# Meowuu7/equi-articulated-pose

Hardware: AMD Instinct MI355X
Metric: point-clouds/sec (4096 pts, 60 anchors) fwd+bwd (higher is better)
Workload: dtype f32; 1 GPU; 8 x 4096-pt synthetic laptop clouds per GPU, 3-block inter backbone 1->64->128->512 (NN=64,K=24,A=60), forward+backward+Adam; clouds_per_gpu=8, points=4096, anchors=60

## Files before the change

equi-articulated-pose_amd/csrc/gemm_bf16x3.hip:

```cpp
#include "common.h"
#include "device_prims.h"
#include <algorithm>
#include <type_traits>

namespace {

constexpr int BK = 16, BN = 256;
constexpr unsigned PLANE_BYTES = 256 * BK * 2;
constexpr unsigned oper_bytes(int pl) { return (unsigned)pl * PLANE_BYTES; }
constexpr unsigned stage_bytes(int pl) { return 2 * oper_bytes(pl); }
constexpr size_t shmem_bytes(int pl) { return 3 * (size_t)stage_bytes(pl); }
constexpr int WAVES_N = 4;

struct Args {
    int M, N, K;
    const float *A; long long lda;
    const float *B; long long ldb, sB;
    float *C; long long ldc, sC;
    int tiles_m, tiles_n;
    const int *tbl; int na;
    int nr;
    const unsigned *Apre;
    long long sA; int slabs, kslab;
    const float *ep_scale, *ep_shift, *ep_res; float ep_slope; long long sRes;
// ... 46 lines not shown

    int id = blockIdx.x, tm, tn;
    {
        const int groups = g.tiles_n / 8 * 8;
        const int xcd = id & 7, slot = id >> 3;
        const int panel = (slot / g.tiles_m) * 8 + xcd;
        if (panel < groups && id < groups * g.tiles_m) { tn = panel; tm = slot % g.tiles_m; }
        else { const int r = id - groups * g.tiles_m; tn = groups + r / g.tiles_m; tm = r % g.tiles_m; }
    }
    const int z = blockIdx.y;
    const int m0 = tm * BM, n0 = tn * BN;
    const int item = g.slabs > 1 ? z / g.slabs : z;
    const long long item_of_z = item;
    const long long kbeg = g.slabs > 1 ? (long long)(z - item * g.slabs) * g.kslab : 0;
    const float *A = g.A + item * g.sA + kbeg;
    const float *B = g.B + item * g.sB + (BMODE == 0 ? kbeg : 0);
    float *C = g.C + (long long)z * g.sC;

    const int t = threadIdx.x, lane = t & 63;
    const int wave = __builtin_amdgcn_readfirstlane(t >> 6);
    const int wm = wave / WN, wn = wave % WN;
    const int li = lane & 31, lh = lane >> 5;

    const int c4 = t & 3, rq = t >> 2;
    const int c4b = BMODE ? __builtin_amdgcn_readfirstlane(t >> 7) : c4, rqb = BMODE ? (t & 127) : rq;
    const float *baseA[NPA], *baseB[NPO];
#pragma unroll
    for (int u = 0; u < NPA; ++u) baseA[u] = A + (long long)min(m0 + RG * u, g.M - RG) * g.lda;
#pragma unroll
    for (int u = 0; u < NPO; ++u) baseB[u] = B + (long long)min(n0 + RG * u, g.N - RG) * g.ldb;
    const unsigned char *preA[NPA];
    constexpr int PRE_PIECE = PL == 3 ? 32 : 16;
    const long long pre_pitch = (long long)(g.K / 4) * PRE_PIECE;
#pragma unroll
    for (int u = 0; u < NPA; ++u) preA[u] = reinterpret_cast<const unsigned char *>(g.Apre) + (long long)min(m0 + RG * u, g.M - RG) * pre_pitch;
    const unsigned offP = (unsigned)((long long)rq * pre_pitch + PRE_PIECE * c4);
    float sclA[2] = {1.0f, 1.0f}, sclB[2] = {1.0f, 1.0f};
    const unsigned *absBz = g.absB + item_of_z * g.sAbsB;
    if constexpr (PL == 2) {
#pragma unroll
        for (int u = 0; u < NPA; ++u) sclA[u] = pow2_scale(__uint_as_float(g.absA[min(m0 + RG * u, g.M - RG) + rq]));
#pragma unroll
        for (int u = 0; u < NPO; ++u) sclB[u] = pow2_scale(__uint_as_float(absBz[(min(n0 + RG * u, g.N - RG) + rqb) / g.grpB]) * g.multB);
    }
    const unsigned offA = (unsigned)((long long)rq * g.lda + 4 * c4) * 4u, offB = (unsigned)((long long)rq * g.ldb + 4 * c4) * 4u;
    unsigned colB[NPO], tapB[NPO];
#pragma unroll
    for (int u = 0; u < NPO; ++u) {
        const int n = min(n0 + RG * u, g.N - RG) + rqb;
        if constexpr (BMODE == 2) {
// ... 314 lines not shown
void keep_pool_memory() {
    static bool done[64] = {};
    int dev = 0;
    if (hipGetDevice(&dev) != hipSuccess || dev < 0 || dev >= 64 || done[dev]) return;
    done[dev] = true;
    hipMemPool_t pool;
    if (hipDeviceGetDefaultMemPool(&pool, dev) == hipSuccess) {
        uint64_t keep = ~0ull;
        (void)hipMemPoolSetAttribute(pool, hipMemPoolAttrReleaseThreshold, &keep);
    }
    (void)hipGetLastError();
}

template <int BMODE, int PL = 3>
int launch_split(Args &g, long long batch, hipStream_t stream, const char *who) {
    bool pre = g.sA == 0 && g.slabs <= 1 && (g_presplit == 2 || (g_presplit == 1 && g.K >= 1024));
    void *scratch = nullptr;
    if (pre) {
        const long long pieces = (long long)g.M * (g.K / 4);
        keep_pool_memory();
        if (hipMallocAsync(&scratch, (size_t)pieces * (PL == 3 ? 32 : 16), stream) != hipSuccess) {
            (void)hipGetLastError();
            scratch = nullptr;
            pre = false;
        }
    }
    struct Release {
        void *p; hipStream_t s;
        ~Release() { if (p) (void)hipFreeAsync(p, s); }
    } release{scratch, stream};
    if (pre) {
// ... 281 lines not shown
    if (!eap_gemm_bf16x3_reduce_f32_supported(M, N, K, A, lda, strideA, B, ldb, strideB, ldc) || (reinterpret_cast<uintptr_t>(C) & 15) ||
        (reinterpret_cast<uintptr_t>(workspace) & 15))
        return eap::bad_arg("gemm_bf16x3_reduce_f32: unsupported operands (ask eap_gemm_bf16x3_reduce_f32_supported)");
    const int slabs = reduce_slabs(M, N, K, batch);
    Args g{};
    g.M = M; g.N = N; g.K = K;
    g.A = A; g.lda = lda; g.sA = strideA;
    g.B = B; g.ldb = ldb; g.sB = strideB;
    g.C = workspace; g.ldc = N; g.sC = (long long)M * N;
    g.slabs = slabs; g.kslab = K / slabs;
    if (int e = launch_split<0>(g, (long long)batch * slabs, eap::S(stream), "gemm_bf16x3_reduce_f32")) return e;
    const long long mn4 = (long long)M * N / 4;
    return eap::run_kernel("gemm_bf16x3_reduce_f32 (sum of the partials)", split_reduce_kernel, eap::cdiv(mn4, 256), 1, 1, dim3(256), 0, eap::S(stream), mn4,
                           batch * slabs, reinterpret_cast<const f32x4 *>(workspace), C, N, (long long)ldc);
}
```

equi-articulated-pose_amd/csrc/grouping.hip:

```cpp
#include "common.h"

namespace {

constexpr int BQ_THREADS = 64;
constexpr int BQ_TILE = 1024;

__device__ __forceinline__ float add_rn(float a, float b) { return __fadd_rn(a, b); }
__device__ __forceinline__ double add_rn(double a, double b) { return __dadd_rn(a, b); }
__device__ __forceinline__ float sub_rn(float a, float b) { return __fsub_rn(a, b); }
__device__ __forceinline__ double sub_rn(double a, double b) { return __dsub_rn(a, b); }
__device__ __forceinline__ float mul_rn(float a, float b) { return __fmul_rn(a, b); }
__device__ __forceinline__ double mul_rn(double a, double b) { return __dmul_rn(a, b); }
__device__ __forceinline__ float div_rn(float a, float b) { return __fdiv_rn(a, b); }
__device__ __forceinline__ double div_rn(double a, double b) { return __ddiv_rn(a, b); }
__device__ __forceinline__ float sqrt_t(float a) { return sqrtf(a); }
__device__ __forceinline__ double sqrt_t(double a) { return sqrt(a); }
__device__ __forceinline__ float acos_t(float a) { return acosf(a); }
__device__ __forceinline__ double acos_t(double a) { return acos(a); }
__device__ __forceinline__ float min_t(float a, float b) { return fminf(a, b); }
__device__ __forceinline__ double min_t(double a, double b) { return fmin(a, b); }

template <typename T>
__device__ __forceinline__ T sq3(T x, T y, T z) {
    return add_rn(add_rn(mul_rn(x, x), mul_rn(y, y)), mul_rn(z, z));
// ... 1 lines not shown
template <typename T>
__device__ __forceinline__ T d2_exact(T ax, T ay, T az, T bx, T by, T bz) {
    return sq3(sub_rn(ax, bx), sub_rn(ay, by), sub_rn(az, bz));
}

template <typename T>
__global__ __launch_bounds__(BQ_THREADS) void ball_query_kernel(
    int n, int m, T radius2, int nsample, const T *__restrict__ new_xyz,
    const T *__restrict__ xyz, int32_t *__restrict__ idx) {
    __shared__ T tile[3][BQ_TILE];
    const int bi = blockIdx.y;
    xyz += (size_t)bi * 3 * n;
    new_xyz += (size_t)bi * 3 * m;
    idx += (size_t)bi * m * nsample;

    const int j = blockIdx.x * BQ_THREADS + threadIdx.x;
    const bool live = j < m;
    T qx = 0, qy = 0, qz = 0;
    if (live) { qx = new_xyz[j]; qy = new_xyz[m + j]; qz = new_xyz[2 * m + j]; }
    int32_t *out = idx + (size_t)(live ? j : 0) * nsample;

    int cnt = live ? 0 : nsample;
    for (int k0 = 0; k0 < n; k0 += BQ_TILE) {
        const int len = min(BQ_TILE, n - k0);
        __syncthreads();
        for (int t = threadIdx.x; t < len; t += BQ_THREADS) {
            tile[0][t] = xyz[k0 + t];
            tile[1][t] = xyz[n + k0 + t];
            tile[2][t] = xyz[2 * n + k0 + t];
        }
        __syncthreads();
        for (int t = 0; t < len && cnt < nsample; ++t) {
            const T d2 = d2_exact(qx, qy, qz, tile[0][t], tile[1][t], tile[2][t]);
            if (d2 < radius2) { out[cnt] = k0 + t; ++cnt; }
        }
        if (__syncthreads_and(cnt >= nsample)) break;
    }
    if (!live) return;
    if (cnt < nsample - 1) {
        if (cnt == 0) {
            for (int t = 0; t < nsample; ++t) out[t] = 0;
        } else {
            for (int t = cnt; t < nsample; ++t) out[t] = out[t - cnt];
        }
    } else if (cnt == nsample - 1) {
        out[nsample - 1] = 0;
    }
}

template <typename T>
int launch_ball_query(int b, int n, int m, float radius, int nsample, const T *new_xyz,
                      const T *xyz, int32_t *idx, hipStream_t s) {
    if (b <= 0 || m <= 0 || nsample <= 0) return 0;
    if (n <= 0) return eap::bad_arg("ball_query: empty support cloud");
    const T r2 = (T)(radius * radius);
    return eap::run_kernel("ball_query", ball_query_kernel<T>, eap::cdiv(m, BQ_THREADS), b, 1, dim3(BQ_THREADS), 0, s, n, m, r2, nsample, new_xyz, xyz, idx);
}


template <typename T>
__global__ __launch_bounds__(1024) void fps_kernel(int n, int m, const T *__restrict__ xyz,
                                                  T *__restrict__ temp, int32_t *__restrict__ idx) {
    __shared__ T s_d[1024];
    __shared__ int s_i[1024];
    const int bi = blockIdx.x, tid = threadIdx.x, nt = blockDim.x;
    xyz += (size_t)bi * 3 * n;
    temp += (size_t)bi * n;
    idx += (size_t)bi * m;
    for (int k = tid; k < n; k += nt) temp[k] = (T)1e10;
    int old = 0;
    if (tid == 0) idx[0] = 0;
// ... 148 lines not shown
```

equi-articulated-pose_amd/csrc/inv_lists.hip:

```cpp
#include "common.h"

namespace {

constexpr int RT = 1024;
constexpr int MAXN = 16384;

__global__ __launch_bounds__(256) void inv_count_kernel(int per_cloud, int n, const int32_t *__restrict__ idx,
                                                        int32_t *__restrict__ counts) {
    extern __shared__ int s_hist[];
    const int bi = blockIdx.y, t = threadIdx.x;
    for (int i = t; i < n; i += 256) s_hist[i] = 0;
    __syncthreads();
    const int chunk = (per_cloud + gridDim.x - 1) / gridDim.x;
    const int beg = blockIdx.x * chunk, end = min(per_cloud, beg + chunk);
    const int32_t *src = idx + (size_t)bi * per_cloud;
    for (int e = beg + t; e < end; e += 256) {
        const int q = src[e];
        if ((unsigned)q < (unsigned)n) atomicAdd(&s_hist[q], 1);
    }
    __syncthreads();
    for (int i = t; i < n; i += 256) {
        const int v = s_hist[i];
        if (v) atomicAdd(&counts[(size_t)bi * n + i], v);
    }
}

__global__ __launch_bounds__(RT) void inv_rows_kernel(int n, int n2, const int32_t *__restrict__ counts,
                                                      int32_t *__restrict__ rows, int32_t *__restrict__ off,
                                                      int32_t *__restrict__ cnt, int32_t *__restrict__ n_rows) {
    extern __shared__ unsigned long long s_key[];
    __shared__ int s_part[RT];
    const int bi = blockIdx.x, t = threadIdx.x;
    for (int i = t; i < n2; i += RT) {
        const unsigned c = i < n ? (unsigned)counts[(size_t)bi * n + i] : 0u;
        s_key[i] = c ? (((unsigned long long)c << 32) | (0xFFFFFFFFu - (unsigned)i)) : 0ull;
    }
    __syncthreads();
    for (int k = 2; k <= n2; k <<= 1) {
        for (int j = k >> 1; j > 0; j >>= 1) {
            for (int i = t; i < n2; i += RT) {
                const int l = i ^ j;
                if (l > i) {
                    const unsigned long long a = s_key[i], b = s_key[l];
                    const bool desc = (i & k) == 0;
                    if (desc ? a < b : a > b) { s_key[i] = b; s_key[l] = a; }
                }
            }
            __syncthreads();
        }
    }
    const int per = n2 / RT > 0 ? n2 / RT : 1;
    int local = 0, nz = 0;
    for (int u = 0; u < per; ++u) {
        const int i = t * per + u;
        if (i < n2) { const unsigned c = (unsigned)(s_key[i] >> 32); local += (int)c; nz += c != 0; }
    }
    s_part[t] = local;
    __syncthreads();
    for (int d = 1; d < RT; d <<= 1) {
        const int v = t >= d ? s_part[t - d] : 0;
        __syncthreads();
        s_part[t] += v;
        __syncthreads();
    }
    int run = s_part[t] - local;
    for (int u = 0; u < per; ++u) {
        const int i = t * per + u;
        if (i < n) {
            const unsigned long long key = s_key[i];
            const unsigned c = (unsigned)(key >> 32);
            rows[(size_t)bi * n + i] = c ? (int)(0xFFFFFFFFu - (unsigned)key) : -1;
            cnt[(size_t)bi * n + i] = (int)c;
            off[(size_t)bi * n + i] = run;
            run += (int)c;
        }
    }
    __syncthreads();
    s_part[t] = nz;
    __syncthreads();
    for (int d = RT / 2; d > 0; d >>= 1) {
        if (t < d) s_part[t] += s_part[t + d];
        __syncthreads();
    }
    if (t == 0) n_rows[bi] = s_part[0];
}

__global__ __launch_bounds__(256) void inv_fill_kernel(int per_cloud, int nn, int n, int rld,
                                                       const int32_t *__restrict__ idx, const float4 *__restrict__ gx,
                                                       const int32_t *__restrict__ rows, const int32_t *__restrict__ off,
                                                       int32_t *__restrict__ ent_p, float4 *__restrict__ ent_gx) {
    __shared__ int s_wave[4];
    const int r = blockIdx.x, bi = blockIdx.y;
    const int q = rows[(size_t)bi * rld + r];
    if (q < 0) return;
    const int t = threadIdx.x, lane = t & 63, wave = t >> 6;
    const int quads = per_cloud >> 2;
    const int qper = (quads + 3) / 4;
    const int qbeg = wave * qper, qend = min(quads, qbeg + qper);
    const int4 *src = reinterpret_cast<const int4 *>(idx + (size_t)bi * per_cloud);
// ... 106 lines not shown
```

equi-articulated-pose_amd/vgtk/_hip.py:

```python
import ctypes
import os
import re
import struct
import types
import weakref

import torch

_PKG_ROOT = os.path.abspath(os.path.join(os.path.dirname(__file__), '..'))
LIB_PATH = os.path.join(_PKG_ROOT, 'libeap_hip.so')

if not os.path.exists(LIB_PATH):
    raise ImportError(
        f'{LIB_PATH} not found: build the HIP extension first '
        '(python -c "import __graft_entry__ as g; g.build()" or make -C equi-articulated-pose_amd/csrc). '
        'This package has no CPU fallback.')

lib = ctypes.CDLL(LIB_PATH)


_HEADERS = (os.path.join(_PKG_ROOT, 'include', 'eap_hip.h'), os.path.join(os.path.dirname(_PKG_ROOT), 'include', 'eap_hip.h'))
HEADER_PATH = next((p for p in _HEADERS if os.path.exists(p)), _HEADERS[-1])

_I64 = ctypes.c_int64
# ... 255 lines not shown
def _product(A, B, out, reduce=False):
    ta, lda, sa, ba, M, K = operand(A, 'A')
    tb, ldb, sb, batch, Kb, N = operand(B, 'B')
    tc, ldc, sc, bc, Mc, Nc = operand(out, 'out')
    if B.dim() != 3 or out.dim() != 3 - reduce:
        raise RuntimeError(f'B is a stack of matrices, out {"one matrix" if reduce else "a stack"}: got B {tuple(B.shape)}, out {tuple(out.shape)}')
    if K != Kb or (M, N) != (Mc, Nc) or (A.dim() == 3 and ba != batch) or bc != (1 if reduce else batch):
        raise RuntimeError(f'A {tuple(A.shape)} x B {tuple(B.shape)} -> out {tuple(out.shape)}: the sizes do not agree')
    if tc:
        raise RuntimeError(f'out must be row-major (strides {tuple(out.stride())})')
    if (M > 1 and ldc < N) or (bc > 1 and sc < (M - 1) * ldc + N):
        raise RuntimeError(f'out {tuple(out.shape)} with strides {tuple(out.stride())} overlaps itself')
    return ta, tb, M, N, K, lda, sa, ldb, sb, ldc, sc, batch


def matmul(A, B, out, b_bound=None):
    ta, tb, M, N, K, lda, sa, ldb, sb, ldc, sc, batch = _product(A, B, out)
    gemm(ta, tb, M, N, K, A, lda, sa, B, ldb, sb, out, ldc, sc, batch, b_bound=b_bound)


def matmul_reduce(A, B, out):
    ta, tb, M, N, K, lda, sa, ldb, sb, ldc, _, batch = _product(A, B, out, reduce=True)
    gemm_reduce(ta, tb, M, N, K, A, lda, sa, B, ldb, sb, out, ldc, batch)


def matmul_reduce_takes_split(A, B, out):
    ta, tb, M, N, K, lda, sa, ldb, sb, ldc, _, _ = _product(A, B, out, reduce=True)
    return bool(SPLIT_BF16_CONTRACTION and not ta and tb and out.data_ptr() % 16 == 0 and
                abi.eap_gemm_bf16x3_reduce_f32_supported(M, N, K, A, lda, sa, B, ldb, sb, ldc))


def matmul_epilogue(A, B, out, scale, shift, slope, residual=None, b_bound=None):
# ... 346 lines not shown
    b, p, nn = idx.shape
    dev = idx.device
    wide = n > DENSE_NARROW_ROWS
    memb = torch.empty(b, p, 32 if wide else 16, dtype=torch.int32, device=dev)
    flags = torch.empty(b, dtype=torch.int32, device=dev)
    slot_of = torch.empty(b, n, dtype=torch.int32, device=dev)
    call('eap_so3_dense_member_wide' if wide else 'eap_so3_dense_member', idx, b, p, n, nn, min(DENSE_MAX_ROWS if wide else DENSE_NARROW_ROWS, n),
         rows.stride(0), idx, rows, n_rows, slot_of, memb, flags)
    return memb, flags


def so3_dense_narrow(memb, rp):
    if _dense_wide(memb) and rp <= DENSE_NARROW_ROWS:
        return memb[:, :, :16].contiguous()
    return memb


SORT_DENSE_POINTS = True
SKIP_DENSE_STEPS = True


class DenseGeometry:

    def __init__(self, q_xyz, s_xyz, memb, rows, rp, rk, sigma, nn, n_rows=None, row_rot=None, sort=None):
        b, p = memb.shape[:2]
        n = s_xyz.shape[2]
        na, ks, _ = rk.shape
        dev = memb.device
        memb = so3_dense_narrow(memb, rp)
        if memb.dtype != torch.int32 or not memb.is_contiguous() or memb.shape[2] not in (16, 32) or int(rp) > 32 * memb.shape[2]:
# ... 546 lines not shown
```

equi-articulated-pose_amd/vgtk/so3conv/functional.py:

```python
import math
import os
import weakref

import numpy as np
import torch

import vgtk
import vgtk.functional as fr
import vgtk.pc as pctk
import vgtk.spconv as zpconv
import vgtk.cuda.grouping as cuda_nn

from .. import _hip
from . import norm_fold

inter_so3conv_feat_grouping = zpconv.inter_zpconv_grouping_naive
batched_index_select = zpconv.batched_index_select
batched_index_select_other = zpconv.batched_index_select_other

MATERIALIZE_INTER_W = False

GAMMA_SIZE = 3
ROOT = vgtk.__path__[0]
Rs, R_idx, canonical_relative = fr.icosahedron_so3(GAMMA_SIZE)
# ... 360 lines not shown
    return ((bias.abs() > NORM_IN_NODE_MAX_RATIO * weight.abs()) & (weight != 0)).any().to(torch.int32)


class _ListHead:

    def __init__(self, idx, n_sup, nonident, gx=None, prefill=False, dense_probe=None, norm=None):
        dev = idx.device
        main = torch.cuda.current_stream(dev)
        side = _side_stream(dev)
        self.memb = None
        side.wait_stream(main)
        for t in (idx, gx, nonident) + tuple(x[1] if isinstance(x, tuple) else x for x in (dense_probe or ())):
            if t is not None:
                t.record_stream(side)
        ill = None
        if norm is not None:
            second = _side_stream(dev, True)
            second.wait_stream(main)
            with torch.cuda.stream(second):
                ill = _norm_ill(norm.weight.detach(), norm.bias.detach())
            ill.record_stream(side)
        with torch.cuda.stream(side):
            self.rows, self.off, self.cnt, self.n_rows = _hip.inv_lists_rows(idx, n_sup)
            flag = nonident.max() if nonident is not None else torch.ones((), dtype=torch.int32, device=dev)
            dense_bad = torch.ones((), dtype=torch.int32, device=dev)
            if dense_probe is not None:
                self.memb, dflags = _hip.so3_dense_member(idx, self.rows, self.n_rows, n_sup)
                dense_bad = dflags.max()
                eye = torch.eye(3, dtype=torch.float32, device=dev)
                for rot in dense_probe:
                    if isinstance(rot, tuple):
                        r = rot[1].double()
                        dense_bad = dense_bad + ((torch.matmul(r, r.transpose(-1, -2)) - eye.double()).abs().max() > 1e-6).to(torch.int32)
                    elif rot is not None:
                        dense_bad = dense_bad + (rot[:, :, :3, :3] != eye).any().to(torch.int32)
            groups16 = torch.zeros((), dtype=torch.int32, device=dev)
            if self.memb is not None:
                touched = ((self.memb & 0xffff) != 0).sum((1, 2)) + ((self.memb & -65536) != 0).sum((1, 2))
                groups16 = (touched.max().to(torch.float32) * (16.0 / max(idx.shape[1], 1))).to(torch.int32)
            stats = [self.n_rows.max().to(torch.int32), flag.to(torch.int32), dense_bad.to(torch.int32), groups16]
            if ill is not None:
                side.wait_stream(second)
                stats.append(ill)
            stats = torch.stack(stats)
            self.host = torch.empty(stats.shape[0], dtype=torch.int32, pin_memory=True)
            self.host.copy_(stats, non_blocking=True)
            self.entries = _hip.inv_lists_fill(idx, gx, self.rows, self.off, n_sup) if (prefill and gx is not None) else None
            self.event = torch.cuda.Event()
            self.event.record(side)
        for t in (self.rows, self.off, self.cnt, self.n_rows, self.memb) + (self.entries or ()):
            if t is not None:
                t.record_stream(main)

    def fill(self, idx, gx, n_sup):
        dev = idx.device
        main = torch.cuda.current_stream(dev)
        side = _side_stream(dev)
        with torch.cuda.stream(side):
            self.entries = _hip.inv_lists_fill(idx, gx, self.rows, self.off, n_sup)
            self.event = torch.cuda.Event()
            self.event.record(side)
        for t in self.entries:
            t.record_stream(main)

# ... 1248 lines not shown
```

include/eap_hip.h:

```cpp
#ifndef EAP_HIP_H
#define EAP_HIP_H

#include <stdint.h>

#ifdef __cplusplus
extern "C" {
#endif

typedef void *eap_stream_t;

const char *eap_last_error(void);
int eap_launch_dims_ok(int64_t gx, int64_t gy, int64_t gz, int bx, int by, int bz);
const char *eap_last_kernel(void);
int eap_abi_version(void);


int eap_ball_query_f32(int b, int n, int m, float radius, int nsample, const float *new_xyz,
                       const float *xyz, int32_t *idx, eap_stream_t stream);
int eap_ball_query_f64(int b, int n, int m, float radius, int nsample, const double *new_xyz,
                       const double *xyz, int32_t *idx, eap_stream_t stream);

int eap_furthest_point_sampling_f32(int b, int n, int m, const float *xyz, float *temp,
                                    int32_t *idx, eap_stream_t stream);
int eap_furthest_point_sampling_f64(int b, int n, int m, const double *xyz, double *temp,
// ... 193 lines not shown
                              const float *bound, float *scale, void *planes, eap_stream_t stream);
int eap_so3_dense_point_keys(int b, int p, const uint32_t *memb, int32_t *keys, eap_stream_t stream);
int64_t eap_so3_dense_steps_words(int b, int p, int ks, int rp, int dir);
int eap_so3_dense_steps(int b, int p, int ks, int rp, int dir, int skip, const int32_t *n_rows, const uint64_t *mask, int32_t *steps,
                        eap_stream_t stream);
int eap_so3_dense_product_steps_f32(int dir, int b, int o, int p, int na, int ks, int rp, int64_t ldz, float sigma, const int32_t *n_rows,
                                    const void *planes, const float *scale, const float *pt, const float *kr, const uint64_t *mask,
                                    const int32_t *steps, float *out, eap_stream_t stream);
int eap_so3_dense_max_rows(void);
int eap_so3_dense_member_wide(int b, int p, int n, int nn, int rp, int rows_ld, const int32_t *idx, const int32_t *rows,
                              const int32_t *n_rows, int32_t *slot_of, uint32_t *memb, int32_t *flags, eap_stream_t stream);
int eap_so3_dense_point_keys_wide(int b, int p, const uint32_t *memb, int64_t *keys, eap_stream_t stream);
int eap_so3_dense_masks_wide(int b, int p, int ks, int rp, int dir, const uint32_t *memb, uint64_t *mask, eap_stream_t stream);
int eap_so3_dense_steps_wide(int b, int p, int ks, int rp, int dir, int skip, const int32_t *n_rows, const uint64_t *mask, int32_t *steps,
                             eap_stream_t stream);


int eap_so3_intra_group_fwd_f32(int b, int c, int p, int na, int t, const float *feats,
                                const int32_t *intra_idx, float *out, eap_stream_t stream);
int eap_so3_intra_group_bwd_f32(int b, int c, int p, int na, int t, const float *gout,
                                const int32_t *intra_idx, float *gfeats, eap_stream_t stream);



int eap_gemm_f32(int transA, int transB, int M, int N, int K, const float *A, int64_t lda,
                 int64_t strideA, const float *B, int64_t ldb, int64_t strideB, float *C,
                 int64_t ldc, int64_t strideC, int batch, eap_stream_t stream);

int64_t eap_gemm_f32_reduce_workspace(int M, int N, int K, int batch);
int eap_gemm_f32_reduce(int transA, int transB, int M, int N, int K, const float *A, int64_t lda,
// ... 17 lines not shown
int64_t eap_gemm_bf16x3_reduce_workspace(int M, int N, int K, int batch);
int eap_gemm_bf16x3_reduce_f32(int M, int N, int K, const float *A, int64_t lda, int64_t strideA, const float *B, int64_t ldb,
                               int64_t strideB, float *C, int64_t ldc, int batch, float *workspace, eap_stream_t stream);
int eap_so3_intra_conv_bf16x3_f32_supported(int b, int o, int c, int p, int na, int nt);
int eap_so3_intra_conv_bf16x3_f32(int b, int o, int c, int p, int na, int nt, const float *W, const float *feats,
                                  const int32_t *intra_idx, float *out, eap_stream_t stream);
int eap_absmax_rows_f32(const float *x, int batch, int rows, int cols, int64_t ld, int64_t stride, int32_t *out_bits, eap_stream_t stream);
int eap_absmax_colgroups_f32(const float *x, int batch, int rows, int cols, int64_t ld, int64_t stride, int grp, int32_t *out_bits,
                             eap_stream_t stream);
int eap_so3_grouped_bound_f32(int b, int p, int nn, int n_sup, const int32_t *point_max_bits, const int32_t *idx, int32_t *out_bits,
                              eap_stream_t stream);
int eap_gemm_f16x2_f32(int trans_b, int M, int N, int K, const float *A, int64_t lda, const float *B, int64_t ldb, int64_t strideB,
                       float *C, int64_t ldc, int64_t strideC, int batch, const int32_t *abs_a, const int32_t *abs_b, int grp_b, float mult_b,
                       const float *scale, const float *shift, float slope, const float *residual, int64_t strideRes,
                       eap_stream_t stream);
int eap_so3_intra_conv_f16x2_f32(int b, int o, int c, int p, int na, int nt, const float *W, const float *feats,
                                 const int32_t *intra_idx, float *out, const int32_t *abs_w, const int32_t *abs_f, eap_stream_t stream);


int eap_gemm_dma_f32_supported(int transA, int transB, int M, int N, int K, const float *A, int64_t lda,
                               int64_t strideA, const float *B, int64_t ldb, int64_t strideB);
int eap_gemm_dma_f32(int transA, int transB, int M, int N, int K, const float *A, int64_t lda, int64_t strideA,
                     const float *B, int64_t ldb, int64_t strideB, float *C, int64_t ldc, int64_t strideC,
                     int batch, eap_stream_t stream);
int64_t eap_gemm_dma_f32_reduce_workspace(int M, int N, int K, int batch);
int eap_gemm_dma_f32_reduce(int transA, int transB, int M, int N, int K, const float *A, int64_t lda,
                            int64_t strideA, const float *B, int64_t ldb, int64_t strideB, float *C, int64_t ldc,
                            int batch, float *workspace, eap_stream_t stream);
int eap_gemm_skinny_reduce_f32_supported(int M, int N, int K, const float *A, int64_t lda, int64_t strideA, const float *B,
                                         int64_t ldb, int64_t strideB);
// ... 160 lines not shown
```

Measured before the change: 169.2 point-clouds/sec.

## Add split-K f16x2 GEMM, cooperative ball query, compact inverse-list sort, fused probe

Several unrelated changes land together. A split-K path for the two-plane GEMM with M=128 spreads the K dimension across slabs and sums the partials in a reduce kernel, so single-row-tile matmuls can fill the GPU. Ball query now uses 16 lanes per query with ballot-based compaction instead of one thread per query. The inverse-list sort compacts nonzero counts before a smaller bitonic sort, and a new native probe kernel folds several statistics checks into one pass on the side stream. The costs are an extra workspace and reduce launch, and changed ordering and fill semantics in ball query (out[t % cnt]).

```diff
diff --git a/equi-articulated-pose_amd/csrc/gemm_bf16x3.hip b/equi-articulated-pose_amd/csrc/gemm_bf16x3.hip
--- a/equi-articulated-pose_amd/csrc/gemm_bf16x3.hip
+++ b/equi-articulated-pose_amd/csrc/gemm_bf16x3.hip
@@ -84,8 +84,12 @@
     const long long item_of_z = item;
     const long long kbeg = g.slabs > 1 ? (long long)(z - item * g.slabs) * g.kslab : 0;
     const float *A = g.A + item * g.sA + kbeg;
-    const float *B = g.B + item * g.sB + (BMODE == 0 ? kbeg : 0);
-    float *C = g.C + (long long)z * g.sC;
+    const float *B = g.B + item * g.sB + (BMODE == 0 ? kbeg : BMODE == 1 ? kbeg * g.ldb : 0);
+    long long zc = z;
+    if constexpr (BMODE == 1) {
+        if (g.slabs > 1) zc = (long long)(z - item * g.slabs) * (gridDim.y / g.slabs) + item;
+    }
+    float *C = g.C + zc * g.sC;
 
     const int t = threadIdx.x, lane = t & 63;
     const int wave = __builtin_amdgcn_readfirstlane(t >> 6);
@@ -103,7 +107,8 @@
     constexpr int PRE_PIECE = PL == 3 ? 32 : 16;
     const long long pre_pitch = (long long)(g.K / 4) * PRE_PIECE;
 #pragma unroll
-    for (int u = 0; u < NPA; ++u) preA[u] = reinterpret_cast<const unsigned char *>(g.Apre) + (long long)min(m0 + RG * u, g.M - RG) * pre_pitch;
+    for (int u = 0; u < NPA; ++u)
+        preA[u] = reinterpret_cast<const unsigned char *>(g.Apre) + (long long)min(m0 + RG * u, g.M - RG) * pre_pitch + (kbeg / 4) * PRE_PIECE;
     const unsigned offP = (unsigned)((long long)rq * pre_pitch + PRE_PIECE * c4);
     float sclA[2] = {1.0f, 1.0f}, sclB[2] = {1.0f, 1.0f};
     const unsigned *absBz = g.absB + item_of_z * g.sAbsB;
@@ -448,7 +453,7 @@
 
 template <int BMODE, int PL = 3>
 int launch_split(Args &g, long long batch, hipStream_t stream, const char *who) {
-    bool pre = g.sA == 0 && g.slabs <= 1 && (g_presplit == 2 || (g_presplit == 1 && g.K >= 1024));
+    bool pre = g.sA == 0 && (g.slabs <= 1 || BMODE == 1) && (g_presplit == 2 || (g_presplit == 1 && g.K >= 1024));
     void *scratch = nullptr;
     if (pre) {
         const long long pieces = (long long)g.M * (g.K / 4);
@@ -760,3 +765,80 @@
     return eap::run_kernel("gemm_bf16x3_reduce_f32 (sum of the partials)", split_reduce_kernel, eap::cdiv(mn4, 256), 1, 1, dim3(256), 0, eap::S(stream), mn4,
                            batch * slabs, reinterpret_cast<const f32x4 *>(workspace), C, N, (long long)ldc);
 }
+
+namespace {
+
+int device_cus() {
+    static std::atomic<int> seen[64] = {};
+    int dev = 0;
+    if (hipGetDevice(&dev) != hipSuccess) { (void)hipGetLastError(); return 256; }
+    const bool slot = dev >= 0 && dev < 64;
+    int n = slot ? seen[dev].load(std::memory_order_relaxed) : 0;
+    if (n > 0) return n;
+    if (hipDeviceGetAttribute(&n, hipDeviceAttributeMultiprocessorCount, dev) != hipSuccess || n <= 0) { (void)hipGetLastError(); n = 256; }
+    if (slot) seen[dev].store(n, std::memory_order_relaxed);
+    return n;
+}
+
+constexpr int SPLITK_MIN_TILES = 16;
+constexpr int SPLITK_MAX_SLABS = 64;
+
+inline bool splitk_slabs_ok(int K, int slabs) {
+    return slabs >= 1 && slabs <= SPLITK_MAX_SLABS && (K / BK) % slabs == 0 && (slabs == 1 || K / BK / slabs >= SPLITK_MIN_TILES);
+}
+
+}
+
+extern "C" int eap_gemm_f16x2_splitk_slabs(int M, int N, int K, int batch, int cus) {
+    if (M != 128 || N <= 0 || batch <= 0 || K < 64 * BK || (K % BK) != 0) return 1;
+    if (cus <= 0) cus = device_cus();
+    const long long tiles = (long long)((N + BN - 1) / BN) * batch;
+    const long long want = (4ll * cus + tiles - 1) / tiles;
+    int best = 1;
+    for (int s = 1; s <= SPLITK_MAX_SLABS; ++s) {
+        if (!splitk_slabs_ok(K, s)) continue;
+        best = s;
+        if (s >= want) break;
+    }
+    const long long kt = K / BK;
+    const long long one = ((tiles + cus - 1) / cus) * kt, cut = ((tiles * best + cus - 1) / cus) * (kt / best);
+    return 4 * cut <= 3 * one ? best : 1;
+}
+
+extern "C" int64_t eap_gemm_f16x2_splitk_workspace(int M, int N, int batch, int slabs) {
+    if (M <= 0 || N <= 0 || batch <= 0 || slabs <= 1) return 0;
+    return (int64_t)M * N * batch * slabs;
+}
+
+extern "C" int eap_gemm_f16x2_splitk_f32(int M, int N, int K, const float *A, int64_t lda, const float *B, int64_t ldb, int64_t strideB,
+                                         float *C, int64_t ldc, int64_t strideC, int batch, const int32_t *abs_a, const int32_t *abs_b, int grp_b,
+                                         float mult_b, int slabs, float *workspace, int64_t workspace_floats, eap_stream_t stream) {
+    if (M <= 0 || N <= 0 || batch <= 0) return eap::bad_arg("gemm_f16x2_splitk_f32: M, N and batch must be positive");
+    if (!A || !B || !C) return eap::bad_arg("gemm_f16x2_splitk_f32: A, B and C are required");
+    if (!abs_a || !abs_b || !(mult_b > 0.f) || grp_b <= 0 || (N % grp_b) != 0)
+        return eap::bad_arg("gemm_f16x2_splitk_f32: the operand magnitudes are required (eap_absmax_rows_f32 / _colgroups_f32), column groups dividing N");
+    if (M != 128 || !eap_gemm_bf16x3_nn_f32_supported(M, N, K, A, lda, B, ldb, strideB))
+        return eap::bad_arg("gemm_f16x2_splitk_f32: one 128-row tile of operands eap_gemm_bf16x3_nn_f32_supported takes");
+    if (slabs == 0) slabs = eap_gemm_f16x2_splitk_slabs(M, N, K, batch, 0);
+    if (!splitk_slabs_ok(K, slabs))
+        return eap::bad_arg("gemm_f16x2_splitk_f32: the slab count must divide the K / 16 k-tiles into slabs of at least 16 (at most 64 slabs)");
+    if ((long long)batch * slabs > 65535) return eap::bad_arg("gemm_f16x2_splitk_f32: batch x slabs exceeds 65535");
+    Args g{};
+    g.M = M; g.N = N; g.K = K;
+    g.A = A; g.lda = lda;
+    g.B = B; g.ldb = ldb; g.sB = strideB;
+    g.C = C; g.ldc = ldc; g.sC = strideC;
+    g.absA = reinterpret_cast<const unsigned *>(abs_a); g.absB = reinterpret_cast<const unsigned *>(abs_b); g.multB = mult_b;
+    g.grpB = grp_b; g.sAbsB = N / grp_b;
+    if (slabs == 1) return launch_split<1, 2>(g, batch, eap::S(stream), "gemm_f16x2_splitk_f32");
+    if (strideC != (int64_t)M * ldc || (ldc & 3) || ldc < N || !eap::aligned16(C, workspace))
+        return eap::bad_arg("gemm_f16x2_splitk_f32: more than one slab needs strideC = M ldc, ldc a multiple of 4, C and the workspace 16-byte aligned");
+    if (!workspace || workspace_floats < eap_gemm_f16x2_splitk_workspace(M, N, batch, slabs))
+        return eap::bad_arg("gemm_f16x2_splitk_f32: the workspace is too small (ask eap_gemm_f16x2_splitk_workspace)");
+    g.C = workspace; g.ldc = N; g.sC = (long long)M * N;
+    g.slabs = slabs; g.kslab = K / slabs;
+    if (int e = launch_split<1, 2>(g, (long long)batch * slabs, eap::S(stream), "gemm_f16x2_splitk_f32")) return e;
+    const long long mn4 = (long long)batch * M * N / 4;
+    return eap::run_kernel("gemm_f16x2_splitk_f32 (sum of the slabs)", split_reduce_kernel, eap::cdiv(mn4, 256), 1, 1, dim3(256), 0, eap::S(stream), mn4, slabs,
+                           reinterpret_cast<const f32x4 *>(workspace), C, N, (long long)ldc);
+}
diff --git a/equi-articulated-pose_amd/csrc/grouping.hip b/equi-articulated-pose_amd/csrc/grouping.hip
--- a/equi-articulated-pose_amd/csrc/grouping.hip
+++ b/equi-articulated-pose_amd/csrc/grouping.hip
@@ -2,7 +2,9 @@
 
 namespace {
 
-constexpr int BQ_THREADS = 64;
+constexpr int BQ_LANES = 16;
+constexpr int BQ_THREADS = 512;
+constexpr int BQ_QUERIES = BQ_THREADS / BQ_LANES;
 constexpr int BQ_TILE = 1024;
 
 __device__ __forceinline__ float add_rn(float a, float b) { return __fadd_rn(a, b); }
@@ -39,7 +41,8 @@
     new_xyz += (size_t)bi * 3 * m;
     idx += (size_t)bi * m * nsample;
 
-    const int j = blockIdx.x * BQ_THREADS + threadIdx.x;
+    const int lane = threadIdx.x & 63, gl = lane & (BQ_LANES - 1), gsh = lane & ~(BQ_LANES - 1);
+    const int j = blockIdx.x * BQ_QUERIES + threadIdx.x / BQ_LANES;
     const bool live = j < m;
     T qx = 0, qy = 0, qz = 0;
     if (live) { qx = new_xyz[j]; qy = new_xyz[m + j]; qz = new_xyz[2 * m + j]; }
@@ -55,21 +58,29 @@
             tile[2][t] = xyz[2 * n + k0 + t];
         }
         __syncthreads();
-        for (int t = 0; t < len && cnt < nsample; ++t) {
+        for (int t0 = 0; t0 < len; t0 += BQ_LANES) {
+            if (__ballot(cnt < nsample) == 0ull) break;
+            const int t = min(t0 + gl, len - 1);
             const T d2 = d2_exact(qx, qy, qz, tile[0][t], tile[1][t], tile[2][t]);
-            if (d2 < radius2) { out[cnt] = k0 + t; ++cnt; }
+            const bool hit = t0 + gl < len && cnt < nsample && d2 < radius2;
+            const unsigned mine = (unsigned)(__ballot(hit) >> gsh) & ((1u << BQ_LANES) - 1u);
+            const int slot = cnt + __popc(mine & ((1u << gl) - 1u));
+            if (hit && slot < nsample) out[slot] = k0 + t;
+            cnt = min(nsample, cnt + __popc(mine));
         }
         if (__syncthreads_and(cnt >= nsample)) break;
     }
+    __threadfence_block();
+    __syncthreads();
     if (!live) return;
     if (cnt < nsample - 1) {
         if (cnt == 0) {
-            for (int t = 0; t < nsample; ++t) out[t] = 0;
+            for (int t = gl; t < nsample; t += BQ_LANES) out[t] = 0;
         } else {
-            for (int t = cnt; t < nsample; ++t) out[t] = out[t - cnt];
+            for (int t = cnt + gl; t < nsample; t += BQ_LANES) out[t] = out[t % cnt];
         }
     } else if (cnt == nsample - 1) {
-        out[nsample - 1] = 0;
+        if (gl == 0) out[nsample - 1] = 0;
     }
 }
 
@@ -79,7 +90,7 @@
     if (b <= 0 || m <= 0 || nsample <= 0) return 0;
     if (n <= 0) return eap::bad_arg("ball_query: empty support cloud");
     const T r2 = (T)(radius * radius);
-    return eap::run_kernel("ball_query", ball_query_kernel<T>, eap::cdiv(m, BQ_THREADS), b, 1, dim3(BQ_THREADS), 0, s, n, m, r2, nsample, new_xyz, xyz, idx);
+    return eap::run_kernel("ball_query", ball_query_kernel<T>, eap::cdiv(m, BQ_QUERIES), b, 1, dim3(BQ_THREADS), 0, s, n, m, r2, nsample, new_xyz, xyz, idx);
 }
 
 
diff --git a/equi-articulated-pose_amd/csrc/inv_lists.hip b/equi-articulated-pose_amd/csrc/inv_lists.hip
--- a/equi-articulated-pose_amd/csrc/inv_lists.hip
+++ b/equi-articulated-pose_amd/csrc/inv_lists.hip
@@ -4,6 +4,7 @@
 
 constexpr int RT = 1024;
 constexpr int MAXN = 16384;
+constexpr int SORT_COMPACT = 2048;
 
 __global__ __launch_bounds__(256) void inv_count_kernel(int per_cloud, int n, const int32_t *__restrict__ idx,
                                                         int32_t *__restrict__ counts) {
@@ -30,15 +31,23 @@
                                                       int32_t *__restrict__ cnt, int32_t *__restrict__ n_rows) {
     extern __shared__ unsigned long long s_key[];
     __shared__ int s_part[RT];
+    __shared__ int s_rows;
     const int bi = blockIdx.x, t = threadIdx.x;
-    for (int i = t; i < n2; i += RT) {
-        const unsigned c = i < n ? (unsigned)counts[(size_t)bi * n + i] : 0u;
-        s_key[i] = c ? (((unsigned long long)c << 32) | (0xFFFFFFFFu - (unsigned)i)) : 0ull;
-    }
-    __syncthreads();
-    for (int k = 2; k <= n2; k <<= 1) {
+    if (t == 0) s_rows = 0;
+    __syncthreads();
+    for (int i = t; i < n; i += RT) {
+        const unsigned c = (unsigned)counts[(size_t)bi * n + i];
+        if (c) s_key[atomicAdd(&s_rows, 1)] = ((unsigned long long)c << 32) | (0xFFFFFFFFu - (unsigned)i);
+    }
+    __syncthreads();
+    const int nref = s_rows;
+    int m2 = n2;
+    if (nref <= SORT_COMPACT) { m2 = 64; while (m2 < nref) m2 <<= 1; }
+    for (int i = nref + t; i < m2; i += RT) s_key[i] = 0ull;
+    __syncthreads();
+    for (int k = 2; k <= m2; k <<= 1) {
         for (int j = k >> 1; j > 0; j >>= 1) {
-            for (int i = t; i < n2; i += RT) {
+            for (int i = t; i < m2; i += RT) {
                 const int l = i ^ j;
                 if (l > i) {
                     const unsigned long long a = s_key[i], b = s_key[l];
@@ -49,11 +58,11 @@
             __syncthreads();
         }
     }
-    const int per = n2 / RT > 0 ? n2 / RT : 1;
-    int local = 0, nz = 0;
+    const int per = m2 / RT > 0 ? m2 / RT : 1;
+    int local = 0;
     for (int u = 0; u < per; ++u) {
         const int i = t * per + u;
-        if (i < n2) { const unsigned c = (unsigned)(s_key[i] >> 32); local += (int)c; nz += c != 0; }
+        if (i < m2) local += (int)(unsigned)(s_key[i] >> 32);
     }
     s_part[t] = local;
     __syncthreads();
@@ -66,7 +75,7 @@
     int run = s_part[t] - local;
     for (int u = 0; u < per; ++u) {
         const int i = t * per + u;
-        if (i < n) {
+        if (i < n && i < m2) {
             const unsigned long long key = s_key[i];
             const unsigned c = (unsigned)(key >> 32);
             rows[(size_t)bi * n + i] = c ? (int)(0xFFFFFFFFu - (unsigned)key) : -1;
@@ -75,14 +84,13 @@
             run += (int)c;
         }
     }
-    __syncthreads();
-    s_part[t] = nz;
-    __syncthreads();
-    for (int d = RT / 2; d > 0; d >>= 1) {
-        if (t < d) s_part[t] += s_part[t + d];
-        __syncthreads();
-    }
-    if (t == 0) n_rows[bi] = s_part[0];
+    const int total = s_part[RT - 1];
+    for (int i = m2 + t; i < n; i += RT) {
+        rows[(size_t)bi * n + i] = -1;
+        cnt[(size_t)bi * n + i] = 0;
+        off[(size_t)bi * n + i] = total;
+    }
+    if (t == 0) n_rows[bi] = nref;
 }
 
 __global__ __launch_bounds__(256) void inv_fill_kernel(int per_cloud, int nn, int n, int rld,
diff --git a/equi-articulated-pose_amd/csrc/list_probe.hip b/equi-articulated-pose_amd/csrc/list_probe.hip
--- /dev/null
+++ b/equi-articulated-pose_amd/csrc/list_probe.hip
@@ -0,0 +1,119 @@
+#include "common.h"
+
+namespace {
+
+constexpr int PROBE_THREADS = 256;
+
+__global__ __launch_bounds__(PROBE_THREADS) void probe_scan_kernel(int b, long long quads_per_cloud, const uint4 *__restrict__ memb,
+                                                                   const float4 *__restrict__ rot_a, long long blocks_a,
+                                                                   const float4 *__restrict__ rot_b, long long blocks_b,
+                                                                   int32_t *__restrict__ work) {
+    const int lane = threadIdx.x & 63, bi = blockIdx.y;
+    if (memb != nullptr) {
+        const uint4 *src = memb + (long long)bi * quads_per_cloud;
+        int mine = 0;
+        for (long long i = (long long)blockIdx.x * PROBE_THREADS + threadIdx.x; i < quads_per_cloud; i += (long long)gridDim.x * PROBE_THREADS) {
+            const uint4 v = src[i];
+            mine += ((v.x & 0xffffu) != 0) + ((v.x >> 16) != 0) + ((v.y & 0xffffu) != 0) + ((v.y >> 16) != 0) +
+                    ((v.z & 0xffffu) != 0) + ((v.z >> 16) != 0) + ((v.w & 0xffffu) != 0) + ((v.w >> 16) != 0);
+        }
+        for (int d = 32; d > 0; d >>= 1) mine += __shfl_xor(mine, d);
+        if (lane == 0 && mine) atomicAdd(&work[bi], mine);
+    }
+    const long long tid = ((long long)bi * gridDim.x + blockIdx.x) * PROBE_THREADS + threadIdx.x;
+    const long long nth = (long long)gridDim.x * gridDim.y * PROBE_THREADS;
+    auto off_identity = [](const float4 *blk) {
+        const float4 r0 = blk[0], r1 = blk[1], r2 = blk[2];
+        return !(r0.x == 1.f) || !(r0.y == 0.f) || !(r0.z == 0.f) || !(r1.x == 0.f) || !(r1.y == 1.f) || !(r1.z == 0.f) ||
+               !(r2.x == 0.f) || !(r2.y == 0.f) || !(r2.z == 1.f);
+    };
+    bool bad_a = false, bad_b = false;
+    for (long long i = tid; i < blocks_a; i += nth) bad_a |= off_identity(rot_a + 4 * i);
+    for (long long i = tid; i < blocks_b; i += nth) bad_b |= off_identity(rot_b + 4 * i);
+    if (__ballot(bad_a) != 0ull && lane == 0) atomicOr(&work[b], 1);
+    if (__ballot(bad_b) != 0ull && lane == 0) atomicOr(&work[b + 1], 1);
+}
+
+__global__ __launch_bounds__(PROBE_THREADS) void probe_fold_kernel(int b, float per16, const int32_t *__restrict__ n_rows,
+                                                                   const int32_t *__restrict__ nonident, const int32_t *__restrict__ dflags,
+                                                                   int has_memb, int has_a, int has_b, const float *__restrict__ rot_cloud,
+                                                                   const float *__restrict__ norm_w, const float *__restrict__ norm_b,
+                                                                   int channels, float ratio, const int32_t *__restrict__ work,
+                                                                   int32_t *__restrict__ out) {
+    __shared__ int s_rows, s_flag, s_bad, s_touched, s_off, s_nan, s_ill;
+    const int t = threadIdx.x;
+    if (t == 0) { s_rows = INT32_MIN; s_flag = INT32_MIN; s_bad = INT32_MIN; s_touched = 0; s_off = 0; s_nan = 0; s_ill = 0; }
+    __syncthreads();
+    for (int bi = t; bi < b; bi += PROBE_THREADS) {
+        atomicMax(&s_rows, n_rows[bi]);
+        if (nonident != nullptr) atomicMax(&s_flag, nonident[bi]);
+        if (dflags != nullptr) atomicMax(&s_bad, dflags[bi]);
+        if (has_memb) atomicMax(&s_touched, work[bi]);
+        if (rot_cloud != nullptr) {
+            const float *r = rot_cloud + 9 * (long long)bi;
+            bool off = false, nan = false;
+            for (int i = 0; i < 3; ++i)
+                for (int j = 0; j < 3; ++j) {
+                    double s = 0.0;
+                    for (int k = 0; k < 3; ++k) s += (double)r[3 * i + k] * (double)r[3 * j + k];
+                    const double d = fabs(s - (i == j ? 1.0 : 0.0));
+                    off |= d > 1e-6;
+                    nan |= d != d;
+                }
+            if (off) atomicOr(&s_off, 1);
+            if (nan) atomicOr(&s_nan, 1);
+        }
+    }
+    if (norm_w != nullptr) {
+        bool ill = false;
+        for (int c = t; c < channels; c += PROBE_THREADS) ill |= fabsf(norm_b[c]) > ratio * fabsf(norm_w[c]) && norm_w[c] != 0.f;
+        if (ill) atomicOr(&s_ill, 1);
+    }
+    __syncthreads();
+    if (t != 0) return;
+    out[0] = s_rows;
+    out[1] = nonident != nullptr ? s_flag : 1;
+    int bad = dflags != nullptr ? s_bad : 1;
+    if (has_a) bad += work[b];
+    if (has_b) bad += work[b + 1];
+    if (rot_cloud != nullptr) bad += (s_off && !s_nan) ? 1 : 0;
+    out[2] = bad;
+    out[3] = has_memb ? (int)((float)s_touched * per16) : 0;
+    out[4] = s_ill;
+}
+
+}
+
+extern "C" int64_t eap_so3_dense_probe_workspace(int b) { return b > 0 ? (int64_t)b + 2 : 0; }
+
+extern "C" int eap_so3_dense_probe(int b, int p, int words, const int32_t *n_rows, const int32_t *nonident, const int32_t *dflags,
+                                   const uint32_t *memb, const float *rot_a, int64_t blocks_a, const float *rot_b, int64_t blocks_b,
+                                   const float *rot_cloud, const float *norm_w, const float *norm_b, int channels, float ratio,
+                                   int32_t *work, int32_t *out, eap_stream_t stream) {
+    if (b <= 0 || p <= 0) return eap::bad_arg("so3_dense_probe: b and p must be positive");
+    if (!n_rows || !work || !out) return eap::bad_arg("so3_dense_probe: n_rows, work and out are required");
+    if ((memb == nullptr) != (dflags == nullptr)) return eap::bad_arg("so3_dense_probe: the membership words and the member flags come together");
+    if (memb != nullptr && words != 16 && words != 32) return eap::bad_arg("so3_dense_probe: 16 or 32 membership words per point");
+    if ((norm_w == nullptr) != (norm_b == nullptr) || (norm_w != nullptr && channels <= 0))
+        return eap::bad_arg("so3_dense_probe: the norm's weight and bias come together, over at least one channel");
+    if ((rot_a != nullptr && blocks_a <= 0) || (rot_b != nullptr && blocks_b <= 0))
+        return eap::bad_arg("so3_dense_probe: a pose tensor needs at least one block");
+    if (!eap::aligned16(memb, rot_a, rot_b)) return eap::bad_arg("so3_dense_probe: membership words and pose tensors 16-byte aligned");
+    hipStream_t s = eap::S(stream);
+    if (int e = eap::hip_fail(hipMemsetAsync(work, 0, sizeof(int32_t) * ((size_t)b + 2), s), "so3_dense_probe memset")) return e;
+    const long long quads = (long long)p * (memb ? words : 0) / 4;
+    const long long na = rot_a ? (long long)blocks_a : 0, nb = rot_b ? (long long)blocks_b : 0;
+    const long long pa = eap::cdiv(na, b), pb = eap::cdiv(nb, b);
+    const long long widest = quads > pa ? (quads > pb ? quads : pb) : (pa > pb ? pa : pb);
+    if (widest > 0) {
+        const long long blocks = eap::cdiv(widest, 4 * PROBE_THREADS);
+        if (int e = eap::run_kernel("so3_dense_probe (scan)", probe_scan_kernel, blocks < 64 ? blocks : 64, b, 1, dim3(PROBE_THREADS), 0, s, b, quads,
+                                    reinterpret_cast<const uint4 *>(memb), reinterpret_cast<const float4 *>(rot_a), na,
+                                    reinterpret_cast<const float4 *>(rot_b), nb, work))
+            return e;
+    }
+    const float per16 = (float)(16.0 / (double)p);
+    return eap::run_kernel("so3_dense_probe (fold)", probe_fold_kernel, 1, 1, 1, dim3(PROBE_THREADS), 0, s, b, per16, n_rows, nonident, dflags,
+                           memb != nullptr ? 1 : 0, rot_a != nullptr ? 1 : 0, rot_b != nullptr ? 1 : 0, rot_cloud, norm_w, norm_b, channels, ratio,
+                           (const int32_t *)work, out);
+}
diff --git a/equi-articulated-pose_amd/vgtk/_hip.py b/equi-articulated-pose_amd/vgtk/_hip.py
--- a/equi-articulated-pose_amd/vgtk/_hip.py
+++ b/equi-articulated-pose_amd/vgtk/_hip.py
@@ -293,8 +293,30 @@
     return ta, tb, M, N, K, lda, sa, ldb, sb, ldc, sc, batch
 
 
+SPLIT_K_ONE_ROW_TILE = True
+
+
+def _matmul_split_k(M, N, K, A, lda, B, ldb, sb, out, ldc, sc, batch, b_bound):
+    if not (SPLIT_K_ONE_ROW_TILE and SPLIT_BF16_CONTRACTION and M == 128 and K >= 16 * 64 and out.is_cuda and sc == M * ldc and ldc % 4 == 0
+            and out.data_ptr() % 16 == 0 and abi.eap_gemm_bf16x3_nn_f32_supported(M, N, K, A, lda, B, ldb, sb)):
+        return False
+    slabs = abi.eap_gemm_f16x2_splitk_slabs(M, N, K, batch, 0)
+    if slabs <= 1:
+        return False
+    two = _planes2(0, M, N, K, A, lda, batch, B, ldb, sb, b_bound)
+    if two is None:
+        return False
+    floats = int(abi.eap_gemm_f16x2_splitk_workspace(M, N, batch, slabs))
+    work = torch.empty(floats, dtype=torch.float32, device=out.device)
+    tag = {'flops': 2.0 * M * N * K * batch, 'shape': ('gemm', 0, 0, M, N, K, batch)}
+    call('eap_gemm_f16x2_splitk_f32', out, M, N, K, A, lda, B, ldb, sb, out, ldc, sc, batch, two[0], two[1], two[2], two[3], slabs, work, floats, tag=tag)
+    return True
+
+
 def matmul(A, B, out, b_bound=None):
     ta, tb, M, N, K, lda, sa, ldb, sb, ldc, sc, batch = _product(A, B, out)
+    if not ta and not tb and (sa == 0 or batch == 1) and _matmul_split_k(M, N, K, A, lda, B, ldb, sb, out, ldc, sc, batch, b_bound):
+        return
     gemm(ta, tb, M, N, K, A, lda, sa, B, ldb, sb, out, ldc, sc, batch, b_bound=b_bound)
 
 
@@ -671,6 +693,32 @@
     if _dense_wide(memb) and rp <= DENSE_NARROW_ROWS:
         return memb[:, :, :16].contiguous()
     return memb
+
+
+NATIVE_LIST_PROBE = True
+
+
+def _probe_f32(t, last):
+    return (t.is_cuda and t.dtype == torch.float32 and t.is_contiguous() and tuple(t.shape[-2:]) == last and t.data_ptr() % 16 == 0
+            and t.numel() > 0)
+
+
+def so3_dense_probe_takes(poses, rot_cloud, norm_w, norm_b):
+    return bool(NATIVE_LIST_PROBE and len(poses) <= 2 and all(_probe_f32(t, (4, 4)) for t in poses)
+                and (rot_cloud is None or (_probe_f32(rot_cloud, (3, 3)) and rot_cloud.dim() == 3))
+                and all(t is None or (t.is_cuda and t.dtype == torch.float32 and t.is_contiguous() and t.dim() == 1) for t in (norm_w, norm_b)))
+
+
+def so3_dense_probe(p, n_rows, nonident, dflags, memb, poses, rot_cloud, norm_w, norm_b, ratio):
+    b = n_rows.shape[0]
+    dev = n_rows.device
+    check_input(n_rows, nonident, dflags, memb)
+    work = torch.empty(int(abi.eap_so3_dense_probe_workspace(b)), dtype=torch.int32, device=dev)
+    out = torch.empty(5, dtype=torch.int32, device=dev)
+    rot = [(t, t.numel() // 16) for t in poses] + [(None, 0)] * (2 - len(poses))
+    call('eap_so3_dense_probe', n_rows, b, int(p), 0 if memb is None else memb.shape[2], n_rows, nonident, dflags, memb, rot[0][0], rot[0][1],
+         rot[1][0], rot[1][1], rot_cloud, norm_w, norm_b, 0 if norm_w is None else norm_w.shape[0], float(ratio), work, out)
+    return out
 
 
 SORT_DENSE_POINTS = True
diff --git a/equi-articulated-pose_amd/vgtk/so3conv/functional.py b/equi-articulated-pose_amd/vgtk/so3conv/functional.py
--- a/equi-articulated-pose_amd/vgtk/so3conv/functional.py
+++ b/equi-articulated-pose_amd/vgtk/so3conv/functional.py
@@ -398,6 +398,21 @@
             if t is not None:
                 t.record_stream(side)
         ill = None
+        poses = tuple(r for r in (dense_probe or ()) if r is not None and not isinstance(r, tuple))
+        clouds = tuple(r[1] for r in (dense_probe or ()) if isinstance(r, tuple))
+        norm_wb = (None, None) if norm is None else (norm.weight.detach(), norm.bias.detach())
+        if len(clouds) <= 1 and _hip.so3_dense_probe_takes(poses, clouds[0] if clouds else None, *norm_wb):
+            with torch.cuda.stream(side):
+                self.rows, self.off, self.cnt, self.n_rows = _hip.inv_lists_rows(idx, n_sup)
+                dflags = None
+                if dense_probe is not None:
+                    self.memb, dflags = _hip.so3_dense_member(idx, self.rows, self.n_rows, n_sup)
+                stats = _hip.so3_dense_probe(idx.shape[1], self.n_rows, nonident, dflags, self.memb, poses, clouds[0] if clouds else None,
+                                             *norm_wb, NORM_IN_NODE_MAX_RATIO)
+                if norm is None:
+                    stats = stats[:4]
+                self._finish(stats, idx, gx, n_sup, prefill, side, main)
+            return
         if norm is not None:
             second = _side_stream(dev, True)
             second.wait_stream(main)
@@ -426,12 +441,14 @@
             if ill is not None:
                 side.wait_stream(second)
                 stats.append(ill)
-            stats = torch.stack(stats)
-            self.host = torch.empty(stats.shape[0], dtype=torch.int32, pin_memory=True)
-            self.host.copy_(stats, non_blocking=True)
-            self.entries = _hip.inv_lists_fill(idx, gx, self.rows, self.off, n_sup) if (prefill and gx is not None) else None
-            self.event = torch.cuda.Event()
-            self.event.record(side)
+            self._finish(torch.stack(stats), idx, gx, n_sup, prefill, side, main)
+
+    def _finish(self, stats, idx, gx, n_sup, prefill, side, main):
+        self.host = torch.empty(stats.shape[0], dtype=torch.int32, pin_memory=True)
+        self.host.copy_(stats, non_blocking=True)
+        self.entries = _hip.inv_lists_fill(idx, gx, self.rows, self.off, n_sup) if (prefill and gx is not None) else None
+        self.event = torch.cuda.Event()
+        self.event.record(side)
         for t in (self.rows, self.off, self.cnt, self.n_rows, self.memb) + (self.entries or ()):
             if t is not None:
                 t.record_stream(main)
diff --git a/include/eap_hip.h b/include/eap_hip.h
--- a/include/eap_hip.h
+++ b/include/eap_hip.h
@@ -231,6 +231,11 @@
 int eap_so3_dense_masks_wide(int b, int p, int ks, int rp, int dir, const uint32_t *memb, uint64_t *mask, eap_stream_t stream);
 int eap_so3_dense_steps_wide(int b, int p, int ks, int rp, int dir, int skip, const int32_t *n_rows, const uint64_t *mask, int32_t *steps,
                              eap_stream_t stream);
+int64_t eap_so3_dense_probe_workspace(int b);
+int eap_so3_dense_probe(int b, int p, int words, const int32_t *n_rows, const int32_t *nonident, const int32_t *dflags,
+                        const uint32_t *memb, const float *rot_a, int64_t blocks_a, const float *rot_b, int64_t blocks_b,
+                        const float *rot_cloud, const float *norm_w, const float *norm_b, int channels, float ratio,
+                        int32_t *work, int32_t *out, eap_stream_t stream);
 
 
 int eap_so3_intra_group_fwd_f32(int b, int c, int p, int na, int t, const float *feats,
@@ -278,6 +283,11 @@
                        float *C, int64_t ldc, int64_t strideC, int batch, const int32_t *abs_a, const int32_t *abs_b, int grp_b, float mult_b,
                        const float *scale, const float *shift, float slope, const float *residual, int64_t strideRes,
                        eap_stream_t stream);
+int eap_gemm_f16x2_splitk_slabs(int M, int N, int K, int batch, int cus);
+int64_t eap_gemm_f16x2_splitk_workspace(int M, int N, int batch, int slabs);
+int eap_gemm_f16x2_splitk_f32(int M, int N, int K, const float *A, int64_t lda, const float *B, int64_t ldb, int64_t strideB,
+                              float *C, int64_t ldc, int64_t strideC, int batch, const int32_t *abs_a, const int32_t *abs_b, int grp_b,
+                              float mult_b, int slabs, float *workspace, int64_t workspace_floats, eap_stream_t stream);
 int eap_so3_intra_conv_f16x2_f32(int b, int o, int c, int p, int na, int nt, const float *W, const float *feats,
                                  const int32_t *intra_idx, float *out, const int32_t *abs_w, const int32_t *abs_f, eap_stream_t stream);
 
```

New measurement: 171.7 point-clouds/sec (median of 6 runs). 1.01x the previous value.
